# tlk00/BitMagic

Measured on AMD Instinct MI355X. Metric: Gbits/s + % HBM roofline, 256-way fused AND+COUNT on 1B-bit vectors, higher is better.
Workload: dtype u64; 1 GPU; aggregator pipeline combine_and_sub counts-only: 256-way AND+COUNT, 256 x 1000000000-bit vectors in total, data set A (common 10% OR noise 10%: no early exit); vectors=256, bits_per_vector=1000000000, density_q16=6554, blocks_per_vector=15259, blocks_per_rank=15259, hbm_resident_bytes=32279432448

## Files before the change

bitmagic_amd/csrc/bmx.hip:

```cpp
#include "bmx_internal.h"
#ifdef BMX_DIAG
#include "bmx_diag.h"
#endif
#include "bmx_kernels2.h"
#include "bmx_kernels3.h"
#include "bmx_kernels4.h"
#include "bmx_kernels5.h"
#include "bmx_kernels6.h"
#include "bmx_kernels7.h"
#include "bmx_kernels8.h"
#include "bmx_kernels9.h"
#include "bmx_kernels10.h"
#include "bmx_kernels11.h"
#include "bmx_kernels12.h"
#include "bmx_kernels13.h"
#include "bmx_kernels14.h"
#include "bmx_kernels15.h"

#include <algorithm>
#include <atomic>
#include <chrono>
#include <cstdio>
#include <cstdlib>
#include <cstring>
// ... 635 lines not shown
    memcpy(h.data() + goff, &g, sizeof(g));
    int rc;
    if ((rc = dmalloc(ctx, &d_buf.p, h.size())) || (rc = h2d_staged(ctx, d_buf.p, h.data(), h.size()))) { d_buf.reset(); return rc; }
    *d_midx = (const u32*)d_buf.p; *d_groups = (const CollGroup*)((const char*)d_buf.p + goff);
    return BMX_OK;
}

static bool use_split(const bmx_ctx* ctx, const bmx_pipeline* p, u64 nitems)
{
    if (ctx->pipe_split == 0 || !nitems) return false;
    if (ctx->pipe_split == 1) return nitems <= 65535u * 16u;
    return nitems <= 384u && (u64)p->n_ops >= 24ull * p->ngroups;
}
#define SPLIT_WAVES 8

typedef void (*pipe_bits_fn)(const u64*, const u32*, const u32*, u32, u32, u32, u32, int, u64*);

static u32 pipe_window_cap(u32 wg)
{
    u32 wpb = wg / 64u;
    u32 per_cu = wpb >= 7u ? 1u : 12u / wpb;
    return 256u * per_cu * wpb;
}
static void pipe_plan(const bmx_ctx* ctx, u64 nitems, u32 ngroups, u32& rows, u32& wg, u32& unroll, u32& window)
{
    rows = (u32)ctx->pipe_rows;
    if (!rows) rows = nitems >= 1400u ? 8u : nitems >= 700u ? 4u : nitems >= 350u ? 2u : 1u;
    unroll = ctx->pipe_unroll ? (u32)ctx->pipe_unroll : ((rows >= 4u || !ctx->pipe_nt) ? 4u : 8u);
    u64 n = nitems * (8u / rows);
    wg = (u32)ctx->pipe_wg;
    if (!wg) {
// ... 53 lines not shown
    case 8: return pipe_bits_rows<8>(unroll, nt, wg);
    case 4: return pipe_bits_rows<4>(unroll, nt, wg);
    case 2: return pipe_bits_rows<2>(unroll, nt, wg);
    case 1: return pipe_bits_rows<1>(unroll, nt, wg);
    default: return nullptr;
    }
}

static int ctx_set_tuning(bmx_ctx* ctx, const char* key, int value)
{
    ARGCHK(ctx && key);
    std::string k(key);
    if (k == "pipe_unroll") { ARGCHK(value == 0 || value == 1 || value == 2 || value == 4 || value == 8 || value == 16); ctx->pipe_unroll = value; }
    else if (k == "pipe_rows") { ARGCHK(value == 0 || value == 8 || value == 4 || value == 2 || value == 1); ctx->pipe_rows = value; }
    else if (k == "pipe_nt") ctx->pipe_nt = value != 0;
    else if (k == "pipe_lds") { ARGCHK(value >= 0 && value <= 160 * 1024); ctx->pipe_lds = value; }
    else if (k == "pipe_slots") { ARGCHK(value == 8 || value == 16); ctx->pipe_slots = value; }
    else if (k == "pipe_staged") { ARGCHK(value >= -1 && value <= 1); ctx->pipe_staged = value; }
    else if (k == "pipe_split") { ARGCHK(value >= -1 && value <= 1); ctx->pipe_split = value; }
    else if (k == "pipe_window") { ARGCHK(value >= -1); ctx->pipe_window = value; }
    else if (k == "or_tile") { ARGCHK(value >= 0 && value <= 3); ctx->or_tile = value; }
    else if (k == "or_rows") { ARGCHK(value >= -1 && value <= 1); ctx->or_rows = value; }
    else if (k == "or_depth") { ARGCHK(value == 4 || value == 8); ctx->or_depth = value; }
    else if (k == "direct_cols") { ARGCHK(value >= 0); ctx->direct_cols = value; }
    else if (k == "pair_stream") { ARGCHK(value == -1 || value == 0 || value == 2 || value == 4 || value == 8); ctx->pair_stream = value; }
    else if (k == "pair_wgs") { ARGCHK(value >= 1 && value <= 8); ctx->pair_wgs = value; }
    else if (k == "range_halves") { ARGCHK(value == 0 || value == 1); ctx->range_halves = value; }
    else if (k == "gap_count") { ARGCHK(value >= -1 && value <= 1); ctx->gap_count = value; }
    else if (k == "agg_shape") { ARGCHK(value == 0 || value == 1); ctx->agg_shape = value; }
    else if (k == "and_rows") { ARGCHK(value >= -1 && value <= 1); ctx->and_rows = value; }
// ... 153 lines not shown
    HIPCHK(hipMalloc((void**)&ctx->d_done, FOLD_DONE_WORDS * 4));
    HIPCHK(hipMemsetAsync(ctx->d_done, 0, FOLD_DONE_WORDS * 4, ctx->stream));
    HIPCHK(hipMalloc((void**)&ctx->d_slots2, COUNT_SLOTS * COUNT_SLOT_STRIDE * sizeof(u64)));
    HIPCHK(hipMemsetAsync(ctx->d_slots2, 0, COUNT_SLOTS * COUNT_SLOT_STRIDE * sizeof(u64), ctx->stream));
    HIPCHK(hipMalloc((void**)&ctx->d_done2, FOLD_DONE_WORDS * 4));
    HIPCHK(hipMemsetAsync(ctx->d_done2, 0, FOLD_DONE_WORDS * 4, ctx->stream));
    HIPCHK(hipHostMalloc((void**)&ctx->h_pend, PEND_SLOTS * 8 * sizeof(u64)));
    HIPCHK(hipMalloc((void**)&ctx->d_cursor, 64));
    HIPCHK(hipMemsetAsync(ctx->d_cursor, 0, 64, ctx->stream));
    { int v = 0; if (hipDeviceGetAttribute(&v, hipDeviceAttributeMaxSharedMemoryPerBlock, device) == hipSuccess && v > 0) ctx->max_lds_bytes = (uint32_t)v; else (void)hipGetLastError(); }
    { size_t fr = 0, tot = 0; if (hipMemGetInfo(&fr, &tot) == hipSuccess && fr) ctx->pack_cap = (uint64_t)fr / 4; else (void)hipGetLastError(); }
    if (const char* e = getenv("BMX_DEBUG_REDZONE")) ctx->redzone = atoi(e) != 0;
    if (const char* e = getenv("BMX_PACK_MAX_MB")) { long long mb = atoll(e); if (mb >= 0) ctx->pack_cap = (uint64_t)mb << 20; }
    if (const char* e = getenv("BMX_POOL_MAX_MB")) { long long mb = atoll(e); if (mb >= 0) ctx->pool_cap = (uint64_t)mb << 20; }
    static const char* const env_keys[][2] = {
        {"BMX_PIPE_UNROLL", "pipe_unroll"}, {"BMX_PIPE_ROWS", "pipe_rows"}, {"BMX_PIPE_NT", "pipe_nt"},
        {"BMX_PIPE_WG", "pipe_wg"}, {"BMX_PIPE_WINDOW", "pipe_window"}, {"BMX_PIPE_SPLIT", "pipe_split"}, {"BMX_OR_TILE", "or_tile"}, {"BMX_OR_ROWS", "or_rows"}, {"BMX_OR_DEPTH", "or_depth"}, {"BMX_OR_WINDOW", "or_window"}, {"BMX_DIRECT_COLS", "direct_cols"}, {"BMX_FF_WINDOW", "ff_window"}, {"BMX_GAP_COUNT", "gap_count"}, {"BMX_AND_ROWS", "and_rows"}, {"BMX_AGG_SHAPE", "agg_shape"}, {"BMX_AND_ROWS_WG", "and_rows_wg"}, {"BMX_AND_ROWS_DEPTH", "and_rows_depth"}, {"BMX_AND_ROWS_NT", "and_rows_nt"}, {"BMX_AND_ROWS_IPW", "and_rows_ipw"}, {"BMX_RANGE_HALVES", "range_halves"}, {"BMX_PAIR_STREAM", "pair_stream"}, {"BMX_PAIR_WGS", "pair_wgs"}, {"BMX_RS_LANES", "rs_lanes"}, {"BMX_RS_SELECT_TOP", "rs_select_top"}, {"BMX_RS_SELECT_SEL", "rs_select_sel"}, {"BMX_RS_LINES", "rs_lines"}, {"BMX_RS_SELECT_LINES", "rs_select_lines"}, {"BMX_RS_SDIR_SHIFT", "rs_sdir_shift"}, {"BMX_COLL_SHAPE", "coll_shape"}, {"BMX_COLL_WINDOW", "coll_window"}, {"BMX_COLL_SPLIT", "coll_split"}, {"BMX_COLL_BUILD", "coll_build"}, {"BMX_EQ_BIG", "eq_big"}, {"BMX_PAIR_LOOP", "pair_loop"}, {"BMX_PAIR_NT", "pair_nt"}, {"BMX_EQ_BIG_SHAPE", "eq_big_shape"}, {"BMX_OP2_WGS", "op2_wgs"}, {"BMX_OP2_LOOP", "op2_loop"}, {"BMX_OP2_NT", "op2_nt"}, {"BMX_GAP_PACK", "gap_pack"}, {"BMX_COLL_MEMBERS", "coll_members"}, {"BMX_XCD_SWIZZLE", "xcd_swizzle"}, {"BMX_RANKC_PATH", "rankc_path"}};
    for (auto& kv : env_keys)
        if (const char* e = getenv(kv[0])) (void)ctx_set_tuning(ctx.get(), kv[1], atoi(e));
    g_last_error.clear();
    *out = ctx.release();
    return BMX_OK;
ABI_END }

int bmx_ctx_destroy(bmx_ctx* ctx) { ABI_TRY if (ctx) ctx_release(ctx); return BMX_OK; ABI_END }

int bmx_ctx_set_tuning(bmx_ctx* ctx, const char* key, int value) { ABI_TRY return ctx_set_tuning(ctx, key, value); ABI_END }

int bmx_probe_stream_rw(bmx_ctx* ctx, uint64_t bytes, int sets, int wgs_per_cu, int iters, float* ms_per_pass)
{ ABI_TRY
    ARGCHK(ctx && ms_per_pass && bytes >= 8192 && sets >= 1 && sets <= 8 && wgs_per_cu >= 1 && wgs_per_cu <= 8 && iters >= 1);
// ... 1171 lines not shown
            hipLaunchKernelGGL(HIP_KERNEL_NAME(k_pipe_counts_staged<S>), dim3(nb_to - nb_from), dim3(S * 64), lds, ctx->stream, \
                               (const u64* const*)p->d_udesc, (const u32*)p->d_unblk, p->nplanes, gv ? gv->gmask : (const u32*)p->d_gmask, gv ? gv->gskip : (const u32*)p->d_gskip, \
                               ngroups, nb_from, nb_to - nb_from, ctx->xcd_swz, (u64*)d_counts); } while (0)
            if (ctx->pipe_slots == 8) LAUNCH_STG(8); else LAUNCH_STG(16);
#undef LAUNCH_STG
            KCHK();
            return BMX_OK;
        }
    }
    if (use_split(ctx, p, nitems64)) {
        size_t lds = (size_t)SPLIT_WAVES * 8192;
        auto fn = k_pipe_split<2, SPLIT_WAVES>;
        HIPCHK(hipFuncSetAttribute(reinterpret_cast<const void*>(fn), hipFuncAttributeMaxDynamicSharedMemorySize, (int)lds));
        hipLaunchKernelGGL(fn, dim3((u32)nitems64), dim3(SPLIT_WAVES * 64), lds, ctx->stream,
                           (const u64*)p->d_dmat, row_off, and_n, sub_n, p->col_stride, ngroups, nb_from, nb_to, 0, (u64*)d_counts,
                           0, (uint4*)nullptr, (u64*)nullptr, (BlockStat*)nullptr);
        KCHK();
        return BMX_OK;
    }
    if (!p->has_gap) {
        u32 rows, wg, unroll, window;
        pipe_plan(ctx, nitems64, ngroups, rows, wg, unroll, window);
        u32 parts = 8u / rows;
        if (nitems64 * parts > 0xFFFFFFF0ull) { g_last_error = "too many work items in one run"; return BMX_ERR_RANGE; }
        pipe_bits_fn fn = pipe_bits_kernel(rows, unroll, ctx->pipe_nt != 0, wg);
        if (!fn) { g_last_error = "this (pipe_rows, pipe_unroll, pipe_nt, pipe_wg) shape is not compiled into the library"; return BMX_ERR_BADARG; }
        u32 wpb = wg / 64u;
        u32 ncols = nb_to - nb_from;
        u32 nwin = window ? (ncols + window - 1u) / window : 1u;
        u32 per = (ncols + nwin - 1u) / nwin;
        for (u32 c0 = 0; c0 < ncols; c0 += per) {
            u32 cols = std::min(per, ncols - c0);
            u32 nitems = cols * ngroups * parts, grid = (nitems + wpb - 1) / wpb;
            hipLaunchKernelGGL(fn, dim3(grid), dim3(wg), (size_t)ctx->pipe_lds, ctx->stream,
                               (const u64*)p->d_dmat, row_off, and_n, p->col_stride, ngroups, nb_from + c0, nitems, ctx->xcd_swz, (u64*)d_counts);
            KCHK();
        }
        return BMX_OK;
    }
    if (nitems64 > 0xFFFFFFF0ull) { g_last_error = "too many (column, group) items in one run"; return BMX_ERR_RANGE; }
    if (use_and_rows(ctx, p)) {
        const u32 ipw = ctx->and_rows_ipw > 0 ? (u32)ctx->and_rows_ipw : 1u;
        hipLaunchKernelGGL(and_rows_kernel<AR_COUNT>(ctx), dim3((u32)((nitems64 + ipw - 1u) / ipw)), dim3((u32)ctx->and_rows_wg), 0, ctx->stream,
                           (const u64*)p->d_dmat, row_off, and_n, sub_n, p->col_stride, ngroups, nb_from, (u32)nitems64, ctx->xcd_swz, (u64*)d_counts,
                           (uint4*)nullptr, (u64*)nullptr, (BlockStat*)nullptr, 0u, 0xFFFFFFFFu, and_rows_diag_bits(), ipw);
        KCHK();
        return BMX_OK;
    }
    if (use_gapcount(ctx, p)) {
        size_t lds = (size_t)(16384 * 2 + 2048) * 4;
// ... 870 lines not shown
                               v->d_bits, v->d_desc, st, nb_from, nb_to);
            e = hipGetLastError();
        }
        return e == hipSuccess ? BMX_OK : fail_hip(e, "k_pipe_counts_gapcount", __LINE__);
    }
    if (!p->has_gap && ncols >= 2560u && ctx->pipe_window >= 0 && (ctx->pipe_wg == 0 || ctx->pipe_wg == 640)) {
        const bool s512 = ctx->agg_shape == 1;
        const u32 wpb = s512 ? 8u : 10u, wgs = wpb * 64u;
        const u32 cap = ctx->pipe_window > 0 ? (u32)ctx->pipe_window : pipe_window_cap(wgs);
        u32 nwin = (ncols + cap - 1u) / cap, per = (ncols + nwin - 1u) / nwin;
        per = (per + wpb - 1u) / wpb * wpb;
        for (u32 c0 = 0; c0 < ncols && e == hipSuccess; c0 += per) {
            u32 n = std::min(per, ncols - c0);
            if (s512) hipLaunchKernelGGL(HIP_KERNEL_NAME(k_agg_and_sub<4, 512>), dim3((n + wpb - 1u) / wpb), dim3(512), 0, ctx->stream,
                               rows, an, sn, p->col_stride, std::min(ncols, c0 + n), 1 , 0,
                               v->d_bits, v->d_desc, st, nb_from, nb_to, c0);
            else hipLaunchKernelGGL(HIP_KERNEL_NAME(k_agg_and_sub<3, 640>), dim3((n + wpb - 1u) / wpb), dim3(640), 0, ctx->stream,
                               rows, an, sn, p->col_stride, std::min(ncols, c0 + n), 1 , 0,
                               v->d_bits, v->d_desc, st, nb_from, nb_to, c0);
            e = hipGetLastError();
        }
    } else {
        size_t lds = p->has_gap ? 4 * 2048 * 4 : 0;
        hipLaunchKernelGGL(HIP_KERNEL_NAME(k_agg_and_sub<2, 256>), dim3((ncols + 3) / 4), dim3(256), lds, ctx->stream,
                           rows, an, sn, p->col_stride, ncols, 1, ctx->xcd_swz, v->d_bits, v->d_desc, st, nb_from, nb_to, 0u);
        e = hipGetLastError();
    }
    return e == hipSuccess ? BMX_OK : fail_hip(e, "k_agg_and_sub", __LINE__);
}

extern "C" {

int bmx_agg_and_sub(bmx_ctx* ctx, const bmx_vec* const* src_and, size_t n_and,
                    const bmx_vec* const* src_sub, size_t n_sub, bmx_vec** result, int* any)
{ ABI_TRY
    ARGCHK(ctx && result && (n_and == 0 || src_and) && (n_sub == 0 || src_sub));
    *result = nullptr;
    if (any) *any = 0;
    int rc = set_dev(ctx); if (rc) return rc;
    uint64_t nbits = 0; uint32_t ncols = 0;
// ... 46 lines not shown
            return BMX_OK;
        }
    }
    uint32_t an = (uint32_t)n_and, sn = (uint32_t)n_sub;
    bmx_pipeline* praw = nullptr;
    if ((rc = bmx_pipeline_create(ctx, src_and, &an, src_sub, &sn, 1, &praw))) return rc;
    Owned<bmx_pipeline> p(praw);
    if ((rc = result_begin(ctx, nbits, ncols, &v, &st, &offs))) return rc;
    if (ncols && use_split(ctx, p.get(), ncols)) {
        size_t lds = (size_t)SPLIT_WAVES * 8192;
        auto fn = k_pipe_split<2, SPLIT_WAVES>;
        hipError_t e = hipFuncSetAttribute(reinterpret_cast<const void*>(fn), hipFuncAttributeMaxDynamicSharedMemorySize, (int)lds);
        if (e == hipSuccess) {
            hipLaunchKernelGGL(fn, dim3(ncols), dim3(SPLIT_WAVES * 64), lds, ctx->stream,
                               (const u64*)p->d_dmat, (const u32*)p->d_meta, (const u32*)(p->d_meta + 1), (const u32*)(p->d_meta + 2),
                               p->col_stride, 1u, 0u, ncols, 1, (u64*)nullptr, 1, v->d_bits, v->d_desc, st);
            e = hipGetLastError();
        }
        if (e != hipSuccess) rc = fail_hip(e, "k_pipe_split", __LINE__);
    } else if (ncols) rc = agg_and_sub_launch(ctx, p.get(), 0u, v.get(), st, 0u, 0xFFFFFFFFu);
    if (!rc) rc = result_finish(ctx, v.get(), st, offs);
    p.reset();
    if (rc) return rc;
    if (any) *any = vec_any_block(v.get());
    *result = v.release();
    return BMX_OK;
ABI_END }

static int run_results_impl(bmx_ctx* ctx, bmx_pipeline* p, uint32_t nb_from, uint32_t nb_to, bmx_vec** results_out, uint64_t* counts_out,
                            const bmx_vec* or_target_in, bmx_vec** or_target_out);

// ... 146 lines not shown
        hipError_t e2 = hipStreamSynchronize(ctx->stream);
        d_tab.reset();
        if (rc) return rc;
        if (e != hipSuccess || e2 != hipSuccess) return fail_hip(e != hipSuccess ? e : e2, "bmx_find_first_and_sub", __LINE__);
        if (ctx->h_small[0] != ~0ull) { *found = 1; *idx = ctx->h_small[0]; }
        return BMX_OK;
    }
    bmx_pipeline* praw = nullptr;
    if ((rc = bmx_pipeline_create(ctx, src_and, &an, src_sub, &sn, 1, &praw))) return rc;
    Owned<bmx_pipeline> p(praw);
    hipError_t e = hipMemsetAsync(ctx->d_small, 0xFF, 8, ctx->stream);
    if (e == hipSuccess) {
        size_t lds = p->has_gap ? 4 * 2048 * 4 : 0;
        rc = windows(512u, [&](u32 c0, u32 c1) {
            hipLaunchKernelGGL(HIP_KERNEL_NAME(k_find_first_and_sub<2>), dim3((c1 - c0 + 3) / 4), dim3(256), lds, ctx->stream,
                               p->d_dmat, p->d_meta + 1, p->d_meta + 2, p->col_stride, c0, c1, has_mask, mf, mt, ctx->d_small);
            hipError_t le = hipGetLastError();
            return le == hipSuccess ? BMX_OK : fail_hip(le, "k_find_first_and_sub", __LINE__);
        });
    }
    if (e == hipSuccess && !rc) e = hipMemcpyAsync(ctx->h_small, ctx->d_small, 8, hipMemcpyDeviceToHost, ctx->stream);
    hipError_t e2 = hipStreamSynchronize(ctx->stream);
    p.reset();
    if (rc) return rc;
    if (e != hipSuccess || e2 != hipSuccess) return fail_hip(e != hipSuccess ? e : e2, "bmx_find_first_and_sub", __LINE__);
    if (ctx->h_small[0] != ~0ull) { *found = 1; *idx = ctx->h_small[0]; }
    return BMX_OK;
}

int bmx_agg_and_sub_indices(bmx_ctx* ctx, const bmx_vec* const* src_and, size_t n_and,
                            const bmx_vec* const* src_sub, size_t n_sub, int width, void* out, uint64_t cap, uint64_t* n)
// ... 928 lines not shown
```

bitmagic_amd/csrc/bmx_device.h:

```cpp
#pragma once
#include <hip/hip_runtime.h>
#include <stdint.h>

typedef uint8_t  u8;
typedef uint16_t u16;
typedef uint32_t u32;
typedef uint64_t u64;

#define GMETA(e) ((u32)((e) >> 48) & 0x1FFFu)
#define GMETA_NONE 0xFFFFFFFFu
#define BMX_DESC_KIND(d) ((u32)((d) & 3ull))
#define BMX_DESC_PTR(d)  ((d) & ~3ull)

typedef u32 u32x4 __attribute__((ext_vector_type(4)));
typedef const __attribute__((address_space(1))) u32x4* gcptr4;
typedef __attribute__((address_space(1))) u32x4* gptr4;
typedef const __attribute__((address_space(1))) u16* gcptr16;

template <int ROWS> struct Part { u32x4 r[ROWS]; };
typedef Part<8> Blk;

__device__ __forceinline__ gcptr4 as_gc4(u64 addr) { return (gcptr4)(uintptr_t)addr; }
__device__ __forceinline__ gcptr4 as_gc4(const void* p) { return (gcptr4)(uintptr_t)p; }
__device__ __forceinline__ gptr4 as_g4(void* p) { return (gptr4)(uintptr_t)p; }
// ... 658 lines not shown
#pragma unroll
    for (u32 k = 0; k < 16; ++k) {
        u64 r = mix64(base + (w64 * 16u + k) * 0xD6E8FEB86659FD93ull);
        acc = ((d >> k) & 1u) ? (acc | r) : (acc & r);
    }
    return acc;
}

__device__ __forceinline__ u64 readlane64(u64 v, u32 l)
{
    u32 lo = __builtin_amdgcn_readlane((u32)v, l);
    u32 hi = __builtin_amdgcn_readlane((u32)(v >> 32), l);
    return ((u64)hi << 32) | lo;
}

template <int U, bool NT, int OPK, int ROWS = 8>
__device__ __forceinline__ bool pipe_chain(Part<ROWS>& acc, const u64* __restrict__ plist, u32 n, u32 lane, u32 poff = 0u)
{
    if (n == 0) return false;
    u64 pn[U];
    auto fetch = [&](u32 k) {
#pragma unroll
        for (int u = 0; u < U; ++u) pn[u] = plist[k + u < n ? k + u : n - 1u];
    };
    auto issue = [&](Part<ROWS>* buf) {
#pragma unroll
        for (int u = 0; u < U; ++u) part_load<ROWS, NT>(buf[u], as_gc4(uniform64(pn[u])) + poff, lane);
    };
    auto consume = [&](Part<ROWS>* buf) {
#pragma unroll
        for (int u = 0; u < U; ++u)
#pragma unroll
            for (int i = 0; i < ROWS; ++i) {
                if constexpr (OPK == 0) acc.r[i] &= buf[u].r[i];
                else if constexpr (OPK == 1) acc.r[i] &= ~buf[u].r[i];
                else acc.r[i] |= buf[u].r[i];
            }
        if constexpr (OPK == 2) return part_is_ones<ROWS>(acc); else return part_is_zero<ROWS>(acc);
    };
    Part<ROWS> A[U], B[U];
    u32 k = U;
    fetch(0);
    issue(A);
    fetch(k);
    bool zero;
    do {
        issue(B); fetch(k + U);
        bool z1 = consume(A);
        issue(A); fetch(k + 2 * U);
        bool z2 = consume(B);
        zero = z1 | z2;
        k += 2 * U;
    } while (!zero && k < n + U);
    return zero;
}
```

bitmagic_amd/csrc/bmx_internal.h:

```cpp
#pragma once
#include "../../include/bmx.h"
#include <hip/hip_runtime.h>
#include <stdint.h>

#include <map>
#include <memory>
#include <string>
#include <unordered_map>
#include <vector>

typedef uint8_t  u8;
typedef uint16_t u16;
typedef uint32_t u32;
typedef uint64_t u64;

int bmx_fail_hip(hipError_t e, const char* what, const char* file, int line);
void bmx_set_last_error(const char* msg);
#define HIPCHK(call) do { hipError_t e_ = (call); if (e_ != hipSuccess) return bmx_fail_hip(e_, #call, __FILE__, __LINE__); } while (0)
#define ARGCHK(cond) do { if (!(cond)) { bmx_set_last_error("bad argument: " #cond); return BMX_ERR_BADARG; } } while (0)
#define KCHK() HIPCHK(hipGetLastError())
#define PEND_SLOTS 1024
#include <new>
#include <stdexcept>
int bmx_abi_caught(int kind, const char* what);
// ... 22 lines not shown
    u64* h_small = nullptr;
    char* h_stage = nullptr; size_t stage_off = 0;
    hipEvent_t ev_stage = nullptr;
    std::multimap<size_t, void*> pool_free;
    std::unordered_map<void*, size_t> pool_live;
    uint64_t pool_cached = 0, pool_cap = 16ull << 30;
    struct RzInfo { void* raw; size_t block; size_t bytes; int line; };
    bool redzone = false;
    std::unordered_map<void*, RzInfo> rz_live;
    uint64_t rz_hits = 0; std::string rz_report;
    long long fail_dmalloc_after = -1;
    bool fail_dmalloc_throws = false;
    int pipe_unroll = 0;
    int pipe_rows = 0;
    int pipe_nt = 1;
    int pipe_wg = 0;
    int pipe_window = 0;
    int pipe_staged = -1;
    int pipe_lds = 0;
    int pipe_slots = 16;
    int pipe_split = -1;
    int or_tile = 0;
    int direct_cols = 384;
    int pair_stream = -1;
    int pair_wgs = 1;
    int range_halves = 1;
    int gap_count = -1;
    int agg_shape = 0;
    int and_rows = -1;
    int and_rows_wg = 256;
// ... 140 lines not shown
```

bitmagic_amd/csrc/bmx_kernels.h:

```cpp
#pragma once
#include "bmx_device.h"

#define DESC_MAKE(ptr, kind) ((u64)(uintptr_t)(ptr) | ((u64)(kind) << 62))
#define DESC_K(d) ((u32)((d) >> 62))
#define DESC_P(d) ((d) & 0x0000FFFFFFFFFFFFull)
#define DESC_MAKE_GAP(ptr, len, sbit) (DESC_MAKE(ptr, K_GAP) | ((u64)((((u32)(len)) << 1) | ((u32)(sbit) & 1u)) << 48))
enum { K_NULL = 0, K_FULL = 1, K_BIT = 2, K_GAP = 3 };

#define ROW_EMPTY 1ull
#define ROW_FULL  2ull
#define ROW_ONES  4ull

struct BlockStat { u32 pop; u32 runs; u32 first; u32 kind; };

__global__ __launch_bounds__(256)
void k_generate(u64 seed, u32 vec_id, int with_common, u32 d, u64 nbits, u64* __restrict__ out, u64 nwords64, u64 word0)
{
    u64 i = (u64)blockIdx.x * blockDim.x + threadIdx.x;
    u64 stride = (u64)gridDim.x * blockDim.x;
    for (; i < nwords64; i += stride) {
        u64 w = word0 + i;
        u64 v = gen_word64(seed, vec_id, w, d);
        if (with_common) v |= gen_word64(seed, 0xFFFFFFFFu, w, d);
        u64 bit0 = w * 64u;
// ... 385 lines not shown
    if (pipe_chain<U, true, 1>(acc, ps, nbs, lane)) return;
    if (nga | ngs) {
        blk_to_lds(acc, lds, lane);
        if (nga && gap_apply_list<GAP_AND>(pa + na - 1u, nga, lds, lane)) return;
        if (ngs && gap_apply_list<GAP_SUB>(ps + ns - 1u, ngs, lds, lane)) return;
        blk_from_lds(acc, lds, lane);
    }
    u32 cnt = wave_sum(blk_lane_popcount(acc));
    if (lane == 0 && cnt) atomicAdd(reinterpret_cast<unsigned long long*>(&counts[g]), (unsigned long long)cnt);
}

template <int U, bool NT, int WG = 256, int ROWS = 8>
__global__ __launch_bounds__(WG)
void k_pipe_counts_bits2(const u64* __restrict__ dmat, const u32* __restrict__ row_off,
                         const u32* __restrict__ and_n, u32 col_stride,
                         u32 ngroups, u32 col_from, u32 nitems, int xcd_swz, u64* __restrict__ counts)
{
    constexpr u32 PARTS = 8 / ROWS;
    u32 lane = lane_id(), wave = threadIdx.x >> 6, wpb = blockDim.x >> 6;
    u32 bid = xcd_swz ? xcd_remap(blockIdx.x, gridDim.x) : blockIdx.x;
    u32 item = uniform32(bid * wpb + wave);
    if (item >= nitems) return;
    u32 part = item % PARTS, cg = item / PARTS;
    u32 c = cg / ngroups, g = cg - c * ngroups;
    const u64* row = dmat + (size_t)(col_from + c) * col_stride + row_off[g];
    u64 hdr = uniform64(row[0]), flags = uniform64(row[1]);
    if (flags & ROW_EMPTY) return;
    if (flags & ROW_FULL) { if (lane == 0) atomicAdd(reinterpret_cast<unsigned long long*>(&counts[g]), (unsigned long long)(65536u / PARTS)); return; }
    u32 nba = (u32)(hdr & 0xFFFFu), nbs = (u32)((hdr >> 32) & 0xFFFFu);
    u32 na = uniform32(and_n[g]);
    const u64* pa = row + 2;
    const u64* ps = pa + na;
    const u32 poff = part * ROWS * 64u;
    Part<ROWS> acc;
#pragma unroll
    for (int i = 0; i < ROWS; ++i) acc.r[i] = (u32x4)(~0u);
    if (pipe_chain<U, NT, 0, ROWS>(acc, pa, nba, lane, poff)) return;
    if (pipe_chain<U, NT, 1, ROWS>(acc, ps, nbs, lane, poff)) return;
    u32 cnt = 0;
#pragma unroll
    for (int i = 0; i < ROWS; ++i) {
        cnt += __popcll(((u64)acc.r[i].y << 32) | acc.r[i].x);
        cnt += __popcll(((u64)acc.r[i].w << 32) | acc.r[i].z);
    }
    cnt = wave_sum(cnt);
    if (lane == 0 && cnt) atomicAdd(reinterpret_cast<unsigned long long*>(&counts[g]), (unsigned long long)cnt);
}

#ifdef BMX_DIAG
template <int AUX>
__global__ __launch_bounds__(256)
void k_diag_stream_read_buf(const uint4* __restrict__ buf, u64 nblocks8k, u32 blocks_per_wave, int pattern, int xcd_swz, u64* __restrict__ sink)
{
// ... 68 lines not shown
```

bitmagic_amd/csrc/bmx_kernels2.h:

```cpp
#pragma once
#include "bmx_kernels.h"

enum { ST_OPT = 1, ST_FORCE_BIT = 2, ST_TEST_ZERO = 4, ST_TEST_ONE = 8, ST_FORCE_GAP = 16, ST_GAP_RESULT = 32 };

__device__ __forceinline__ void gap_emit_from_transitions(const Blk& t, u32 len, u32 first, u16* __restrict__ g, u32 lane, u16* __restrict__ stage)
{
    u32 idx_base = 1u;
#pragma unroll
    for (int i = 0; i < 8; ++i) {
        u32 c = __popc(t.r[i].x) + __popc(t.r[i].y) + __popc(t.r[i].z) + __popc(t.r[i].w);
        u32 incl = wave_scan_incl(c, lane);
        u32 idx = idx_base + incl - c;
        u32 wbase = (u32)i * 256u + lane * 4u;
        u32 tw[4] = {t.r[i].x, t.r[i].y, t.r[i].z, t.r[i].w};
#pragma unroll
        for (int j = 0; j < 4; ++j) {
            u32 m = tw[j];
            while (m) {
                u32 k = __builtin_ctz(m); m &= m - 1u;
                stage[idx++] = (u16)((wbase + j) * 32u + k - 1u);
            }
        }
        idx_base += __shfl(incl, 63, 64);
    }
// ... 658 lines not shown
    for (u32 tc = wave; tc < OR_TILE; tc += (blockDim.x >> 6)) {
        u32 c = c0 + tc;
        if (c >= ncols) break;
        if (full[tc]) { store_trivial(K_FULL, c, desc, st, lane); continue; }
        Blk b;
        blk_from_lds(b, lds_dyn + tc * 2048u, lane);
        store_result_mode(b, c, opt_compress ? ST_OPT : ST_FORCE_BIT, slab, desc, st, lane);
    }
}

template <int U, int WG = 256>
__global__ __launch_bounds__(WG)
void k_agg_and_sub(const u64* __restrict__ dmat, const u32* __restrict__ and_n_p, const u32* __restrict__ sub_n_p,
                   u32 col_stride, u32 ncols, int opt_compress, int xcd_swz,
                   uint4* __restrict__ slab, u64* __restrict__ desc, BlockStat* __restrict__ st,
                   u32 col_from, u32 col_to, u32 col_base)
{
    extern __shared__ u32 lds_dyn[];
    u32 lane = lane_id(), wave = threadIdx.x >> 6;
    u32 bid = xcd_swz ? xcd_remap(blockIdx.x, gridDim.x) : blockIdx.x;
    u32 c = uniform32(col_base + bid * (u32)(WG / 64) + wave);
    if (c >= ncols) return;
    if (c < col_from || c >= col_to) { store_trivial(K_NULL, c, desc, st, lane); return; }
    const u64* row = dmat + (size_t)c * col_stride;
    u64 hdr = uniform64(row[0]), flags = uniform64(row[1]);
    if (flags & ROW_EMPTY) { store_trivial(K_NULL, c, desc, st, lane); return; }
    if (flags & ROW_FULL) { store_trivial(K_FULL, c, desc, st, lane); return; }
    u32 nba = (u32)(hdr & 0xFFFFu), nga = (u32)((hdr >> 16) & 0xFFFFu);
    u32 nbs = (u32)((hdr >> 32) & 0xFFFFu), ngs = (u32)(hdr >> 48);
    u32 na = uniform32(and_n_p[0]), ns = uniform32(sub_n_p[0]);
    const u64* pa = row + 2;
    const u64* ps = pa + na;
    u32* lds = lds_dyn + wave * 2048u;
    Blk acc;
    blk_fill(acc, ~0u);
    bool zero = pipe_chain<U, true, 0>(acc, pa, nba, lane);
    if (!zero) zero = pipe_chain<U, true, 1>(acc, ps, nbs, lane);
    if (!zero && (nga | ngs)) {
        blk_to_lds(acc, lds, lane);
        zero = nga && gap_apply_list<GAP_AND>(pa + na - 1u, nga, lds, lane);
        if (!zero) zero = ngs && gap_apply_list<GAP_SUB>(ps + ns - 1u, ngs, lds, lane);
        if (!zero) { blk_from_lds(acc, lds, lane); zero = blk_is_zero(acc); }
    }
    if (zero) { store_trivial(K_NULL, c, desc, st, lane); return; }
    store_result(acc, c, opt_compress, slab, desc, st, lane);
}

template <int U, int SPLIT>
__global__ __launch_bounds__(SPLIT * 64)
void k_pipe_split(const u64* __restrict__ dmat, const u32* __restrict__ row_off, const u32* __restrict__ and_n,
                  const u32* __restrict__ sub_n, u32 col_stride, u32 ngroups, u32 col_from, u32 col_to, int mode,
                  u64* __restrict__ counts, int opt_compress, uint4* __restrict__ slab, u64* __restrict__ desc,
                  BlockStat* __restrict__ st)
{
    extern __shared__ u32 lds_dyn[];
    u32 lane = lane_id(), wave = threadIdx.x >> 6;
    u32 item = blockIdx.x;
    u32 c = col_from + item / ngroups, g = item % ngroups;
    if (mode == 1 && c >= col_to) { if (wave == 0) store_trivial(K_NULL, c, desc, st, lane); return; }
    const u64* row = dmat + (size_t)c * col_stride + row_off[g];
    u64 hdr = uniform64(row[0]), flags = uniform64(row[1]);
    if (flags & ROW_EMPTY) { if (mode == 1 && wave == 0) store_trivial(K_NULL, c, desc, st, lane); return; }
    if (flags & ROW_FULL) {
        if (wave == 0) {
            if (mode == 1) store_trivial(K_FULL, c, desc, st, lane);
            else if (lane == 0) atomicAdd(reinterpret_cast<unsigned long long*>(&counts[g]), 65536ull);
        }
        return;
    }
    u32 nba = (u32)(hdr & 0xFFFFu), nga = (u32)((hdr >> 16) & 0xFFFFu);
    u32 nbs = (u32)((hdr >> 32) & 0xFFFFu), ngs = (u32)(hdr >> 48);
    u32 na = uniform32(and_n[g]), ns = uniform32(sub_n[g]);
    const u64* pa = row + 2;
    const u64* ps = pa + na;
    Blk acc;
    blk_fill(acc, ~0u);
    {
        u32 a0 = (u32)(((u64)nba * wave) / SPLIT), a1 = (u32)(((u64)nba * (wave + 1u)) / SPLIT);
        u32 s0 = (u32)(((u64)nbs * wave) / SPLIT), s1 = (u32)(((u64)nbs * (wave + 1u)) / SPLIT);
        bool zero = pipe_chain<U, false, 0>(acc, pa + a0, a1 - a0, lane);
        if (!zero) zero = pipe_chain<U, false, 1>(acc, ps + s0, s1 - s0, lane);
        if (zero) blk_fill(acc, 0u);
    }
    u32* mine = lds_dyn + wave * 2048u;
    blk_to_lds(acc, mine, lane);
    __syncthreads();
    if (wave != 0) return;
#pragma unroll 1
    for (u32 k = 1; k < (u32)SPLIT; ++k) { Blk t; blk_from_lds(t, lds_dyn + k * 2048u, lane); blk_and(acc, t); }
    bool zero = blk_is_zero(acc);
    if (!zero && (nga | ngs)) {
        blk_to_lds(acc, mine, lane);
        zero = nga && gap_apply_list<GAP_AND>(pa + na - 1u, nga, mine, lane);
        if (!zero) zero = ngs && gap_apply_list<GAP_SUB>(ps + ns - 1u, ngs, mine, lane);
        if (!zero) { blk_from_lds(acc, mine, lane); zero = blk_is_zero(acc); }
    }
// ... 89 lines not shown
    for (int i = 7; i >= 0; --i) {
        u32 w[4] = {acc.r[i].x, acc.r[i].y, acc.r[i].z, acc.r[i].w};
#pragma unroll
        for (int j = 3; j >= 0; --j)
            if (w[j]) mine = (((u32)i * 256u + lane * 4u + (u32)j) << 5) + (u32)__builtin_ctz(w[j]);
    }
#pragma unroll
    for (int o = 32; o > 0; o >>= 1) { u32 t = __shfl_xor(mine, o, 64); mine = t < mine ? t : mine; }
    return mine;
}

template <int U>
__global__ __launch_bounds__(256)
void k_find_first_and_sub(const u64* __restrict__ dmat, const u32* __restrict__ and_n_p, const u32* __restrict__ sub_n_p,
                          u32 col_stride, u32 col_from, u32 ncols, int has_mask, u32 mask_from, u32 mask_to,
                          u64* __restrict__ best)
{
    extern __shared__ u32 lds_dyn[];
    u32 lane = lane_id(), wave = threadIdx.x >> 6;
    u32 c = uniform32(col_from + blockIdx.x * 4u + wave);
    if (c >= ncols) return;
    u64 cur = __hip_atomic_load(best, __ATOMIC_RELAXED, __HIP_MEMORY_SCOPE_AGENT);
    if (((u64)c << 16) > cur) return;
    const u64* row = dmat + (size_t)c * col_stride;
    u64 hdr = uniform64(row[0]), flags = uniform64(row[1]);
    if (flags & ROW_EMPTY) return;
    if (flags & ROW_FULL) { if (lane == 0) atomicMin(reinterpret_cast<unsigned long long*>(best), ((unsigned long long)c << 16) + (has_mask ? mask_from : 0u)); return; }
    u32 nba = (u32)(hdr & 0xFFFFu), nga = (u32)((hdr >> 16) & 0xFFFFu);
    u32 nbs = (u32)((hdr >> 32) & 0xFFFFu), ngs = (u32)(hdr >> 48);
    u32 na = uniform32(and_n_p[0]), ns = uniform32(sub_n_p[0]);
    const u64* pa = row + 2;
    const u64* ps = pa + na;
    u32* lds = lds_dyn + wave * 2048u;
    Blk acc;
    blk_fill(acc, ~0u);
    if (pipe_chain<U, false, 0>(acc, pa, nba, lane)) return;
    if (pipe_chain<U, false, 1>(acc, ps, nbs, lane)) return;
    if (nga | ngs) {
        blk_to_lds(acc, lds, lane);
        if (nga && gap_apply_list<GAP_AND>(pa + na - 1u, nga, lds, lane)) return;
        if (ngs && gap_apply_list<GAP_SUB>(ps + ns - 1u, ngs, lds, lane)) return;
        blk_from_lds(acc, lds, lane);
    }
    if (has_mask) blk_bit_range(acc, mask_from, mask_to, lane);
    u32 mine = blk_first_bit(acc, lane);
    if (lane == 0 && mine != 0xFFFFFFFFu)
        atomicMin(reinterpret_cast<unsigned long long*>(best), ((unsigned long long)c << 16) + mine);
}

#define DIRECT_MAX_OPS 1024u
enum { DIRECT_AND_SUB = 0, DIRECT_FIND_FIRST = 1, DIRECT_OR = 2 };
template <int SPLIT, int MODE>
// ... 516 lines not shown
```

Baseline: 55600 Gbit/s.

## Add narrow-load mode to pipe_chain that fetches only live accumulator lanes

```diff
diff --git a/bitmagic_amd/csrc/bmx.hip b/bitmagic_amd/csrc/bmx.hip
--- a/bitmagic_amd/csrc/bmx.hip
+++ b/bitmagic_amd/csrc/bmx.hip
@@ -673,7 +673,7 @@
 }
 #define SPLIT_WAVES 8
 
-typedef void (*pipe_bits_fn)(const u64*, const u32*, const u32*, u32, u32, u32, u32, int, u64*);
+typedef void (*pipe_bits_fn)(const u64*, const u32*, const u32*, u32, u32, u32, u32, int, u64*, int);
 
 static u32 pipe_window_cap(u32 wg)
 {
@@ -757,6 +757,7 @@
     if (k == "pipe_unroll") { ARGCHK(value == 0 || value == 1 || value == 2 || value == 4 || value == 8 || value == 16); ctx->pipe_unroll = value; }
     else if (k == "pipe_rows") { ARGCHK(value == 0 || value == 8 || value == 4 || value == 2 || value == 1); ctx->pipe_rows = value; }
     else if (k == "pipe_nt") ctx->pipe_nt = value != 0;
+    else if (k == "pipe_narrow") ctx->pipe_narrow = value != 0;
     else if (k == "pipe_lds") { ARGCHK(value >= 0 && value <= 160 * 1024); ctx->pipe_lds = value; }
     else if (k == "pipe_slots") { ARGCHK(value == 8 || value == 16); ctx->pipe_slots = value; }
     else if (k == "pipe_staged") { ARGCHK(value >= -1 && value <= 1); ctx->pipe_staged = value; }
@@ -940,7 +941,7 @@
     if (const char* e = getenv("BMX_PACK_MAX_MB")) { long long mb = atoll(e); if (mb >= 0) ctx->pack_cap = (uint64_t)mb << 20; }
     if (const char* e = getenv("BMX_POOL_MAX_MB")) { long long mb = atoll(e); if (mb >= 0) ctx->pool_cap = (uint64_t)mb << 20; }
     static const char* const env_keys[][2] = {
-        {"BMX_PIPE_UNROLL", "pipe_unroll"}, {"BMX_PIPE_ROWS", "pipe_rows"}, {"BMX_PIPE_NT", "pipe_nt"},
+        {"BMX_PIPE_UNROLL", "pipe_unroll"}, {"BMX_PIPE_ROWS", "pipe_rows"}, {"BMX_PIPE_NT", "pipe_nt"}, {"BMX_PIPE_NARROW", "pipe_narrow"},
         {"BMX_PIPE_WG", "pipe_wg"}, {"BMX_PIPE_WINDOW", "pipe_window"}, {"BMX_PIPE_SPLIT", "pipe_split"}, {"BMX_OR_TILE", "or_tile"}, {"BMX_OR_ROWS", "or_rows"}, {"BMX_OR_DEPTH", "or_depth"}, {"BMX_OR_WINDOW", "or_window"}, {"BMX_DIRECT_COLS", "direct_cols"}, {"BMX_FF_WINDOW", "ff_window"}, {"BMX_GAP_COUNT", "gap_count"}, {"BMX_AND_ROWS", "and_rows"}, {"BMX_AGG_SHAPE", "agg_shape"}, {"BMX_AND_ROWS_WG", "and_rows_wg"}, {"BMX_AND_ROWS_DEPTH", "and_rows_depth"}, {"BMX_AND_ROWS_NT", "and_rows_nt"}, {"BMX_AND_ROWS_IPW", "and_rows_ipw"}, {"BMX_RANGE_HALVES", "range_halves"}, {"BMX_PAIR_STREAM", "pair_stream"}, {"BMX_PAIR_WGS", "pair_wgs"}, {"BMX_RS_LANES", "rs_lanes"}, {"BMX_RS_SELECT_TOP", "rs_select_top"}, {"BMX_RS_SELECT_SEL", "rs_select_sel"}, {"BMX_RS_LINES", "rs_lines"}, {"BMX_RS_SELECT_LINES", "rs_select_lines"}, {"BMX_RS_SDIR_SHIFT", "rs_sdir_shift"}, {"BMX_COLL_SHAPE", "coll_shape"}, {"BMX_COLL_WINDOW", "coll_window"}, {"BMX_COLL_SPLIT", "coll_split"}, {"BMX_COLL_BUILD", "coll_build"}, {"BMX_EQ_BIG", "eq_big"}, {"BMX_PAIR_LOOP", "pair_loop"}, {"BMX_PAIR_NT", "pair_nt"}, {"BMX_EQ_BIG_SHAPE", "eq_big_shape"}, {"BMX_OP2_WGS", "op2_wgs"}, {"BMX_OP2_LOOP", "op2_loop"}, {"BMX_OP2_NT", "op2_nt"}, {"BMX_GAP_PACK", "gap_pack"}, {"BMX_COLL_MEMBERS", "coll_members"}, {"BMX_XCD_SWIZZLE", "xcd_swizzle"}, {"BMX_RANKC_PATH", "rankc_path"}};
     for (auto& kv : env_keys)
         if (const char* e = getenv(kv[0])) (void)ctx_set_tuning(ctx.get(), kv[1], atoi(e));
@@ -2142,7 +2143,7 @@
         HIPCHK(hipFuncSetAttribute(reinterpret_cast<const void*>(fn), hipFuncAttributeMaxDynamicSharedMemorySize, (int)lds));
         hipLaunchKernelGGL(fn, dim3((u32)nitems64), dim3(SPLIT_WAVES * 64), lds, ctx->stream,
                            (const u64*)p->d_dmat, row_off, and_n, sub_n, p->col_stride, ngroups, nb_from, nb_to, 0, (u64*)d_counts,
-                           0, (uint4*)nullptr, (u64*)nullptr, (BlockStat*)nullptr);
+                           0, (uint4*)nullptr, (u64*)nullptr, (BlockStat*)nullptr, ctx->pipe_narrow);
         KCHK();
         return BMX_OK;
     }
@@ -2161,7 +2162,7 @@
             u32 cols = std::min(per, ncols - c0);
             u32 nitems = cols * ngroups * parts, grid = (nitems + wpb - 1) / wpb;
             hipLaunchKernelGGL(fn, dim3(grid), dim3(wg), (size_t)ctx->pipe_lds, ctx->stream,
-                               (const u64*)p->d_dmat, row_off, and_n, p->col_stride, ngroups, nb_from + c0, nitems, ctx->xcd_swz, (u64*)d_counts);
+                               (const u64*)p->d_dmat, row_off, and_n, p->col_stride, ngroups, nb_from + c0, nitems, ctx->xcd_swz, (u64*)d_counts, ctx->pipe_narrow);
             KCHK();
         }
         return BMX_OK;
@@ -3062,16 +3063,16 @@
             u32 n = std::min(per, ncols - c0);
             if (s512) hipLaunchKernelGGL(HIP_KERNEL_NAME(k_agg_and_sub<4, 512>), dim3((n + wpb - 1u) / wpb), dim3(512), 0, ctx->stream,
                                rows, an, sn, p->col_stride, std::min(ncols, c0 + n), 1 , 0,
-                               v->d_bits, v->d_desc, st, nb_from, nb_to, c0);
+                               v->d_bits, v->d_desc, st, nb_from, nb_to, c0, ctx->pipe_narrow);
             else hipLaunchKernelGGL(HIP_KERNEL_NAME(k_agg_and_sub<3, 640>), dim3((n + wpb - 1u) / wpb), dim3(640), 0, ctx->stream,
                                rows, an, sn, p->col_stride, std::min(ncols, c0 + n), 1 , 0,
-                               v->d_bits, v->d_desc, st, nb_from, nb_to, c0);
+                               v->d_bits, v->d_desc, st, nb_from, nb_to, c0, ctx->pipe_narrow);
             e = hipGetLastError();
         }
     } else {
         size_t lds = p->has_gap ? 4 * 2048 * 4 : 0;
         hipLaunchKernelGGL(HIP_KERNEL_NAME(k_agg_and_sub<2, 256>), dim3((ncols + 3) / 4), dim3(256), lds, ctx->stream,
-                           rows, an, sn, p->col_stride, ncols, 1, ctx->xcd_swz, v->d_bits, v->d_desc, st, nb_from, nb_to, 0u);
+                           rows, an, sn, p->col_stride, ncols, 1, ctx->xcd_swz, v->d_bits, v->d_desc, st, nb_from, nb_to, 0u, ctx->pipe_narrow);
         e = hipGetLastError();
     }
     return e == hipSuccess ? BMX_OK : fail_hip(e, "k_agg_and_sub", __LINE__);
@@ -3148,7 +3149,7 @@
         if (e == hipSuccess) {
             hipLaunchKernelGGL(fn, dim3(ncols), dim3(SPLIT_WAVES * 64), lds, ctx->stream,
                                (const u64*)p->d_dmat, (const u32*)p->d_meta, (const u32*)(p->d_meta + 1), (const u32*)(p->d_meta + 2),
-                               p->col_stride, 1u, 0u, ncols, 1, (u64*)nullptr, 1, v->d_bits, v->d_desc, st);
+                               p->col_stride, 1u, 0u, ncols, 1, (u64*)nullptr, 1, v->d_bits, v->d_desc, st, ctx->pipe_narrow);
             e = hipGetLastError();
         }
         if (e != hipSuccess) rc = fail_hip(e, "k_pipe_split", __LINE__);
@@ -3325,7 +3326,7 @@
         size_t lds = p->has_gap ? 4 * 2048 * 4 : 0;
         rc = windows(512u, [&](u32 c0, u32 c1) {
             hipLaunchKernelGGL(HIP_KERNEL_NAME(k_find_first_and_sub<2>), dim3((c1 - c0 + 3) / 4), dim3(256), lds, ctx->stream,
-                               p->d_dmat, p->d_meta + 1, p->d_meta + 2, p->col_stride, c0, c1, has_mask, mf, mt, ctx->d_small);
+                               p->d_dmat, p->d_meta + 1, p->d_meta + 2, p->col_stride, c0, c1, has_mask, mf, mt, ctx->d_small, ctx->pipe_narrow);
             hipError_t le = hipGetLastError();
             return le == hipSuccess ? BMX_OK : fail_hip(le, "k_find_first_and_sub", __LINE__);
         });
diff --git a/bitmagic_amd/csrc/bmx_device.h b/bitmagic_amd/csrc/bmx_device.h
--- a/bitmagic_amd/csrc/bmx_device.h
+++ b/bitmagic_amd/csrc/bmx_device.h
@@ -696,8 +696,35 @@
     return ((u64)hi << 32) | lo;
 }
 
-template <int U, bool NT, int OPK, int ROWS = 8>
-__device__ __forceinline__ bool pipe_chain(Part<ROWS>& acc, const u64* __restrict__ plist, u32 n, u32 lane, u32 poff = 0u)
+#define PIPE_NARROW_DIV 8u
+
+template <int ROWS>
+__device__ __forceinline__ u32 part_live(const Part<ROWS>& b, u64 (&live)[ROWS])
+{
+    u32 t = 0;
+#pragma unroll
+    for (int i = 0; i < ROWS; ++i) {
+        live[i] = __ballot((b.r[i].x | b.r[i].y | b.r[i].z | b.r[i].w) != 0u);
+        t += (u32)__popcll(live[i]);
+    }
+    return t;
+}
+template <int ROWS>
+__device__ __forceinline__ void part_narrow_offsets(const Part<ROWS>& b, const u64 (&live)[ROWS], u32 lane, u32 (&boff)[ROWS])
+{
+    u32 first = 0u;
+#pragma unroll
+    for (int i = ROWS - 1; i >= 0; --i) first = live[i] ? (u32)i * 64u + (u32)__builtin_ctzll(live[i]) : first;
+#pragma unroll
+    for (int i = 0; i < ROWS; ++i) {
+        u32 row = live[i] ? (u32)i * 64u + (u32)__builtin_ctzll(live[i]) : first;
+        bool mine = (b.r[i].x | b.r[i].y | b.r[i].z | b.r[i].w) != 0u;
+        boff[i] = (mine ? (u32)i * 64u + lane : row) << 4;
+    }
+}
+
+template <int U, bool NT, int OPK, int ROWS = 8, int NARROW = 2>
+__device__ __forceinline__ bool pipe_chain(Part<ROWS>& acc, const u64* __restrict__ plist, u32 n, u32 lane, u32 poff = 0u, int narrow = 0)
 {
     if (n == 0) return false;
     u64 pn[U];
@@ -709,30 +736,86 @@
 #pragma unroll
         for (int u = 0; u < U; ++u) part_load<ROWS, NT>(buf[u], as_gc4(uniform64(pn[u])) + poff, lane);
     };
+    auto consume1 = [&](const Part<ROWS>& b) {
+#pragma unroll
+        for (int i = 0; i < ROWS; ++i) {
+            if constexpr (OPK == 0) acc.r[i] &= b.r[i];
+            else if constexpr (OPK == 1) acc.r[i] &= ~b.r[i];
+            else acc.r[i] |= b.r[i];
+        }
+    };
     auto consume = [&](Part<ROWS>* buf) {
 #pragma unroll
-        for (int u = 0; u < U; ++u)
-#pragma unroll
-            for (int i = 0; i < ROWS; ++i) {
-                if constexpr (OPK == 0) acc.r[i] &= buf[u].r[i];
-                else if constexpr (OPK == 1) acc.r[i] &= ~buf[u].r[i];
-                else acc.r[i] |= buf[u].r[i];
-            }
-        if constexpr (OPK == 2) return part_is_ones<ROWS>(acc); else return part_is_zero<ROWS>(acc);
+        for (int u = 0; u < U; ++u) consume1(buf[u]);
+    };
+    auto saturated = [&]() { if constexpr (OPK == 2) return part_is_ones<ROWS>(acc); else return part_is_zero<ROWS>(acc); };
+    auto steady = [&](Part<ROWS>* X, Part<ROWS>* Y, u32 k) {
+        bool zero;
+        do {
+            issue(Y); fetch(k + U);
+            consume(X); bool z1 = saturated();
+            issue(X); fetch(k + 2 * U);
+            consume(Y); bool z2 = saturated();
+            zero = z1 | z2;
+            k += 2 * U;
+        } while (!zero && k < n + U);
+        return zero;
     };
     Part<ROWS> A[U], B[U];
-    u32 k = U;
+    u32 k = 0u;
     fetch(0);
+    if constexpr (OPK != 2 && NARROW != 0) {
+        if (narrow) {
+            u64 live[ROWS];
+            u32 boff[ROWS];
+            auto load_n = [&](Part<ROWS>& b, u64 p, u32 po) {
+                const __attribute__((address_space(1))) char* base = (const __attribute__((address_space(1))) char*)(as_gc4(uniform64(p)) + po);
+#pragma unroll
+                for (int i = 0; i < ROWS; ++i) {
+                    if constexpr (NT) b.r[i] = __builtin_nontemporal_load((gcptr4)(base + boff[i]));
+                    else b.r[i] = *(gcptr4)(base + boff[i]);
+                }
+            };
+            constexpr int H = (ROWS >= 8 || U == 1) ? 1 : (U * ROWS > 8 ? (8 / ROWS < U ? 8 / ROWS : U) : U);
+            auto fold_batch = [&](bool sparse) {
+                u32 po = poff;
+#pragma unroll
+                for (int h = 0; h < U; h += H) {
+#pragma unroll
+                    for (int u = h; u < h + H; ++u) {
+                        if (sparse) load_n(A[u], pn[u], po);
+                        else part_load<ROWS, NT>(A[u], as_gc4(uniform64(pn[u])) + po, lane);
+                    }
+#pragma unroll
+                    for (int u = h; u < h + H; ++u) consume1(A[u]);
+                    if (h + H < U) asm volatile("" : "+s"(po) : "v"(acc.r[0].x));
+                }
+            };
+            u32 t = part_live<ROWS>(acc, live);
+            if (t == 0u) return true;
+            if (t > (u32)ROWS * 64u / PIPE_NARROW_DIV) {
+                fold_batch(false);
+                fetch(U);
+                k = U;
+                t = part_live<ROWS>(acc, live);
+                if (t == 0u) return true;
+                if (n <= (u32)U) return false;
+            }
+            if (NARROW >= 2 && t <= (u32)ROWS * 64u / PIPE_NARROW_DIV) {
+                do {
+                    u32 l = lane;
+                    asm volatile("" : "+v"(l));
+                    part_narrow_offsets<ROWS>(acc, live, l, boff);
+                    fold_batch(true);
+                    fetch(k + U);
+                    t = part_live<ROWS>(acc, live);
+                    k += U;
+                } while (t != 0u && k < n);
+                return t == 0u;
+            }
+        }
+    }
     issue(A);
-    fetch(k);
-    bool zero;
-    do {
-        issue(B); fetch(k + U);
-        bool z1 = consume(A);
-        issue(A); fetch(k + 2 * U);
-        bool z2 = consume(B);
-        zero = z1 | z2;
-        k += 2 * U;
-    } while (!zero && k < n + U);
-    return zero;
-}
+    fetch(k + U);
+    return steady(A, B, k + U);
+}
diff --git a/bitmagic_amd/csrc/bmx_internal.h b/bitmagic_amd/csrc/bmx_internal.h
--- a/bitmagic_amd/csrc/bmx_internal.h
+++ b/bitmagic_amd/csrc/bmx_internal.h
@@ -60,6 +60,7 @@
     int pipe_unroll = 0;
     int pipe_rows = 0;
     int pipe_nt = 1;
+    int pipe_narrow = 1;
     int pipe_wg = 0;
     int pipe_window = 0;
     int pipe_staged = -1;
diff --git a/bitmagic_amd/csrc/bmx_kernels.h b/bitmagic_amd/csrc/bmx_kernels.h
--- a/bitmagic_amd/csrc/bmx_kernels.h
+++ b/bitmagic_amd/csrc/bmx_kernels.h
@@ -423,7 +423,7 @@
 __global__ __launch_bounds__(WG)
 void k_pipe_counts_bits2(const u64* __restrict__ dmat, const u32* __restrict__ row_off,
                          const u32* __restrict__ and_n, u32 col_stride,
-                         u32 ngroups, u32 col_from, u32 nitems, int xcd_swz, u64* __restrict__ counts)
+                         u32 ngroups, u32 col_from, u32 nitems, int xcd_swz, u64* __restrict__ counts, int narrow)
 {
     constexpr u32 PARTS = 8 / ROWS;
     u32 lane = lane_id(), wave = threadIdx.x >> 6, wpb = blockDim.x >> 6;
@@ -441,11 +441,12 @@
     const u64* pa = row + 2;
     const u64* ps = pa + na;
     const u32 poff = part * ROWS * 64u;
+    constexpr int LVL = (U == 8 && ROWS == 4) ? 0 : 2;
     Part<ROWS> acc;
 #pragma unroll
     for (int i = 0; i < ROWS; ++i) acc.r[i] = (u32x4)(~0u);
-    if (pipe_chain<U, NT, 0, ROWS>(acc, pa, nba, lane, poff)) return;
-    if (pipe_chain<U, NT, 1, ROWS>(acc, ps, nbs, lane, poff)) return;
+    if (pipe_chain<U, NT, 0, ROWS, LVL>(acc, pa, nba, lane, poff, narrow)) return;
+    if (pipe_chain<U, NT, 1, ROWS, LVL>(acc, ps, nbs, lane, poff, narrow)) return;
     u32 cnt = 0;
 #pragma unroll
     for (int i = 0; i < ROWS; ++i) {
diff --git a/bitmagic_amd/csrc/bmx_kernels2.h b/bitmagic_amd/csrc/bmx_kernels2.h
--- a/bitmagic_amd/csrc/bmx_kernels2.h
+++ b/bitmagic_amd/csrc/bmx_kernels2.h
@@ -696,7 +696,7 @@
 void k_agg_and_sub(const u64* __restrict__ dmat, const u32* __restrict__ and_n_p, const u32* __restrict__ sub_n_p,
                    u32 col_stride, u32 ncols, int opt_compress, int xcd_swz,
                    uint4* __restrict__ slab, u64* __restrict__ desc, BlockStat* __restrict__ st,
-                   u32 col_from, u32 col_to, u32 col_base)
+                   u32 col_from, u32 col_to, u32 col_base, int narrow)
 {
     extern __shared__ u32 lds_dyn[];
     u32 lane = lane_id(), wave = threadIdx.x >> 6;
@@ -714,10 +714,11 @@
     const u64* pa = row + 2;
     const u64* ps = pa + na;
     u32* lds = lds_dyn + wave * 2048u;
+    constexpr int AGG_NARROW = (U == 3 && WG == 640) ? 1 : WG == 256 ? 0 : 2;
     Blk acc;
     blk_fill(acc, ~0u);
-    bool zero = pipe_chain<U, true, 0>(acc, pa, nba, lane);
-    if (!zero) zero = pipe_chain<U, true, 1>(acc, ps, nbs, lane);
+    bool zero = pipe_chain<U, true, 0, 8, AGG_NARROW>(acc, pa, nba, lane, 0u, narrow);
+    if (!zero) zero = pipe_chain<U, true, 1, 8, AGG_NARROW>(acc, ps, nbs, lane, 0u, narrow);
     if (!zero && (nga | ngs)) {
         blk_to_lds(acc, lds, lane);
         zero = nga && gap_apply_list<GAP_AND>(pa + na - 1u, nga, lds, lane);
@@ -733,7 +734,7 @@
 void k_pipe_split(const u64* __restrict__ dmat, const u32* __restrict__ row_off, const u32* __restrict__ and_n,
                   const u32* __restrict__ sub_n, u32 col_stride, u32 ngroups, u32 col_from, u32 col_to, int mode,
                   u64* __restrict__ counts, int opt_compress, uint4* __restrict__ slab, u64* __restrict__ desc,
-                  BlockStat* __restrict__ st)
+                  BlockStat* __restrict__ st, int narrow)
 {
     extern __shared__ u32 lds_dyn[];
     u32 lane = lane_id(), wave = threadIdx.x >> 6;
@@ -760,8 +761,8 @@
     {
         u32 a0 = (u32)(((u64)nba * wave) / SPLIT), a1 = (u32)(((u64)nba * (wave + 1u)) / SPLIT);
         u32 s0 = (u32)(((u64)nbs * wave) / SPLIT), s1 = (u32)(((u64)nbs * (wave + 1u)) / SPLIT);
-        bool zero = pipe_chain<U, false, 0>(acc, pa + a0, a1 - a0, lane);
-        if (!zero) zero = pipe_chain<U, false, 1>(acc, ps + s0, s1 - s0, lane);
+        bool zero = pipe_chain<U, false, 0>(acc, pa + a0, a1 - a0, lane, 0u, narrow);
+        if (!zero) zero = pipe_chain<U, false, 1>(acc, ps + s0, s1 - s0, lane, 0u, narrow);
         if (zero) blk_fill(acc, 0u);
     }
     u32* mine = lds_dyn + wave * 2048u;
@@ -881,7 +882,7 @@
 __global__ __launch_bounds__(256)
 void k_find_first_and_sub(const u64* __restrict__ dmat, const u32* __restrict__ and_n_p, const u32* __restrict__ sub_n_p,
                           u32 col_stride, u32 col_from, u32 ncols, int has_mask, u32 mask_from, u32 mask_to,
-                          u64* __restrict__ best)
+                          u64* __restrict__ best, int narrow)
 {
     extern __shared__ u32 lds_dyn[];
     u32 lane = lane_id(), wave = threadIdx.x >> 6;
@@ -901,8 +902,8 @@
     u32* lds = lds_dyn + wave * 2048u;
     Blk acc;
     blk_fill(acc, ~0u);
-    if (pipe_chain<U, false, 0>(acc, pa, nba, lane)) return;
-    if (pipe_chain<U, false, 1>(acc, ps, nbs, lane)) return;
+    if (pipe_chain<U, false, 0>(acc, pa, nba, lane, 0u, narrow)) return;
+    if (pipe_chain<U, false, 1>(acc, ps, nbs, lane, 0u, narrow)) return;
     if (nga | ngs) {
         blk_to_lds(acc, lds, lane);
         if (nga && gap_apply_list<GAP_AND>(pa + na - 1u, nga, lds, lane)) return;
```

Result: slower. 49320 Gbit/s (-11.3%).
